# dremovd/PPO

Hardware: AMD Instinct MI355X
Metric: env-steps/sec (Pong-shaped synthetic, 256 envs/GPU) (higher is better)
Workload: dtype f32

## Files before the change

include/ppo_amd.h:

```cpp
#ifndef PPO_AMD_H
#define PPO_AMD_H

#include <stddef.h>
#include <stdint.h>

#ifdef __cplusplus
extern "C" {
#endif

#define PPO_OK 0
#define PPO_E_INVALID (-1)
#define PPO_E_HIP (-2)
#define PPO_E_ALIGN (-3)

#define PPO_TERM_NONE 0
#define PPO_TERM_U8 1
#define PPO_TERM_F32 2

#define PPO_SCAN_AUTO 0
#define PPO_SCAN_COLUMNS 1
#define PPO_SCAN_TILES 2

int ppo_version(void);
const char *ppo_last_error(void);
// ... 177 lines not shown
                      void *stream);
int ppo_accumulate_f32(float *dst, const float *src, int64_t n, void *stream);
int ppo_mask_mul_f32(float *w, const uint8_t *mask, int64_t n, void *stream);

size_t ppo_tvf_returns_workspace_bytes(int N, int A, int ND, int K, int C);
int ppo_tvf_returns_f32(const float *rewards, const uint8_t *dones, const float *value_samples, int N, int A, int V,
                        int K, int C, double gamma, const int32_t *n_eff, const int32_t *nd_index,
                        const int32_t *nd_of_n, int max_n, int ND, const int32_t *main_plan, const double *main_w,
                        const int32_t *tail_plan, const double *tail_w, const uint8_t *k_zero, void *workspace,
                        size_t workspace_bytes, float *out, void *stream);

int ppo_impala_stack_tail_supported(int channels, int h, int w);
int ppo_impala_stack_tail_forward_f32(const float *in, const float *const *packed_weights, const float *const *biases,
                                      float *a0, float *q0, float *a1, float *q1, int n_images, int channels, int h,
                                      int w, void *stream);
int ppo_impala_stack_tail_backward_f32(const float *g, const float *const *packed_weights_t, const float *const *masks,
                                       float *da1, float *g1, float *da0, float *g0, int n_images, int channels,
                                       int h, int w, void *stream);

int ppo_impala_stack_full_supported(int channels, int h, int w);
int ppo_impala_stack_chain_forward_f32(const float *in, const float *const *pre_packed_weights,
                                       const float *const *pre_biases, float *pre_a0, float *pre_q0, float *pre_a1,
                                       float *pre_q1, const float *const *packed_weights, const float *const *biases,
                                       float *pooled, uint8_t *argmax, float *a0, float *q0, float *a1, float *q1,
                                       int n_images, int channels, int h, int w, void *stream);
size_t ppo_impala_stack_chain_split_workspace_bytes(int n_images, int channels, int h, int w);
int ppo_impala_stack_chain_split_forward_f32(const float *in, const float *const *pre_packed_weights,
                                             const float *const *pre_biases, const float *const *packed_weights,
                                             const float *const *biases, float *q1, void *workspace, size_t workspace_bytes,
                                             int n_images, int channels, int h, int w, void *stream);
int ppo_impala_stack_full_backward_f32(const float *g, const float *const *packed_weights_t, const float *const *masks,
                                       const uint8_t *argmax, float *da1, float *g1, float *da0, float *g0, float *dc,
                                       float *g_prev, int n_images, int channels, int h, int w, void *stream);
int ppo_impala_stack_full_forward_f32(const float *in, const float *const *packed_weights, const float *const *biases,
                                      float *pooled, uint8_t *argmax, float *a0, float *q0, float *a1, float *q1,
                                      int n_images, int channels, int h, int w, void *stream);

int ppo_obs_moments_f64(const void *x, int is_u8, int B, int F, double *moments, void *stream);
int ppo_obs_rms_update_f64(const double *moments, double batch_count, double count, double *mean, double *var,
                           float *mu, float *std, int F, void *stream);
int ppo_obs_normalize_f32(const void *x, int is_u8, const float *mu, const float *std, float eps, float *out, int B,
                          int F, void *stream);

void *ppo_synth_env_create(int n_envs, int64_t obs_bytes, uint64_t seed, double p_done, int64_t env_offset,
                           int n_threads);
void ppo_synth_env_destroy(void *env);
int ppo_synth_env_reset(void *env, uint8_t *obs_out);
int ppo_synth_env_step(void *env, const int32_t *actions, uint8_t *obs_out, float *reward_out, uint8_t *done_out,
                       int32_t *time_out, float *ep_score_out, int32_t *ep_len_out);
int ppo_synth_env_step_upload(void *env, const int32_t *actions, uint8_t *obs_out, float *reward_out, uint8_t *done_out,
                              int32_t *time_out, float *ep_score_out, int32_t *ep_len_out, void *obs_dev, int n_chunks,
                              void *stream);
int ppo_synth_env_get_state(void *env, int64_t *steps_out, int32_t *time_out, float *score_out);
int ppo_synth_env_set_state(void *env, const int64_t *steps, const int32_t *time, const float *score, uint8_t *obs_out);

typedef struct ppo_mlp_net {
    const float *w1, *b1;
    const float *w2, *b2;
    const float *wh, *bh;
    int F, H, NH;
    int act;
} ppo_mlp_net;
typedef struct ppo_mlp_grads {
    float *dw1, *db1, *dw2, *db2, *dwh, *dbh;
    float *dlog_std;
    int n_log_std;
// ... 78 lines not shown
```

ppo_amd/_lib.py:

```python
import ctypes
import os
import threading

HERE = os.path.dirname(os.path.abspath(__file__))
LIB_PATH = os.environ.get("PPO_AMD_LIB") or os.path.join(HERE, "lib", "libppo_amd.so")

PPO_TERM_NONE, PPO_TERM_U8, PPO_TERM_F32 = 0, 1, 2
PPO_SCAN_AUTO, PPO_SCAN_COLUMNS, PPO_SCAN_TILES = 0, 1, 2
PPO_IN_NONE, PPO_IN_RELU, PPO_IN_U8 = 0, 1, 2

_vp = ctypes.c_void_p
_i = ctypes.c_int
_i64 = ctypes.c_int64
_d = ctypes.c_double
_f = ctypes.c_float
_sz = ctypes.c_size_t
_u64 = ctypes.c_uint64

SIGNATURES = {
    "ppo_version": (_i, []),
    "ppo_last_error": (ctypes.c_char_p, []),
    "ppo_gae_scan_f32": (_i, [_vp, _vp, _vp, _vp, _i, _vp, _vp, _i, _i, _i64, _d, _d, _d, _i, _vp]),
    "ppo_bootstrapped_returns_f32": (_i, [_vp, _vp, _i, _vp, _vp, _d, _vp, _i, _i, _i64, _vp]),
    "ppo_conv3x3_forward_f32": (_i, [_vp, _i, _vp, _vp, _vp, _vp, _i, _i, _i, _i, _i, _vp]),
# ... 28 lines not shown
    "ppo_synth_env_step_upload": (_i, [_vp, _vp, _vp, _vp, _vp, _vp, _vp, _vp, _vp, _i, _vp]),
    "ppo_synth_env_get_state": (_i, [_vp, _vp, _vp, _vp]),
    "ppo_synth_env_set_state": (_i, [_vp, _vp, _vp, _vp, _vp]),
    "ppo_ppo_loss_f32": (_i, [_vp, _i, _i, _i, _i, _vp, _vp, _vp, _vp, _vp, _f, _f, _f, _f, _vp, _vp, _vp, _vp]),
    "ppo_conv3x3_pool_forward_f32": (_i, [_vp, _i, _vp, _vp, _vp, _vp, _i, _i, _i, _i, _i, _vp]),
    "ppo_conv3x3_packed_floats": (_sz, [_i, _i, _i]),
    "ppo_conv3x3_pack_weights_f32": (_i, [_vp, _i, _vp]),
    "ppo_conv3x3_forward_packed_f32": (_i, [_vp, _i, _vp, _vp, _vp, _vp, _i, _i, _i, _i, _i, _vp]),
    "ppo_conv3x3_backward_data_packed_f32": (_i, [_vp, _vp, _vp, _vp, _vp, _i, _i, _i, _i, _i, _vp]),
    "ppo_conv3x3_pool_forward_packed_f32": (_i, [_vp, _i, _vp, _vp, _vp, _vp, _i, _i, _i, _i, _i, _vp]),
    "ppo_conv3x3_pool_forward_packed_indexed_f32": (_i, [_vp, _vp, _i, _vp, _vp, _vp, _vp, _i, _i, _i, _i, _i, _vp]),
    "ppo_conv1_pool_form": (_i, [_i]),
    "ppo_conv3x3_block_supported": (_i, [_i, _i, _i]),
    "ppo_conv3x3_block_forward_packed_f32": (_i, [_vp, _vp, _vp, _vp, _vp, _vp, _i, _i, _i, _i, _vp]),
    "ppo_conv3x3_backward_weight_slabs_f32": (_i, [_vp, _i, _vp, _vp, _sz, _i, _i, _i, _i, _i, _vp, _vp]),
    "ppo_conv3x3_backward_weight_pooled_supported": (_i, [_i, _i, _i, _i]),
    "ppo_conv3x3_backward_weight_slabs_pooled_f32": (_i, [_vp, _i, _vp, _vp, _vp, _sz, _i, _i, _i, _i, _i, _vp, _vp]),
    "ppo_conv3x3_backward_weight_slabs_pooled_indexed_f32": (_i, [_vp, _vp, _i, _vp, _vp, _vp, _sz, _i, _i, _i, _i, _i, _vp, _vp]),
    "ppo_conv3x3_backward_weight_slabs_batch_f32": (_i, [_vp, _i, _vp, _vp, _sz, _i, _i, _i, _i, _i, _i, _vp, _vp]),
    "ppo_conv3x3_backward_weight_slabs_batch_mixed_f32": (_i, [_vp, _vp, _vp, _vp, _sz, _i, _i, _i, _i, _i, _i, _vp, _vp]),
    "ppo_conv3x3_backward_weight_bf16x3_supported": (_i, [_i, _i, _i, _i]),
    "ppo_conv3x3_backward_weight_slabs_batch_bf16x3": (_i, [_vp, _vp, _vp, _vp, _sz, _i, _i, _i, _i, _i, _i, _vp, _vp]),
    "ppo_conv3x3_wgrad_reduce_f32": (_i, [_vp, _i, _vp]),
    "ppo_tanh_forward_f32": (_i, [_vp, _vp, _sz, _vp]),
    "ppo_tanh_backward_f32": (_i, [_vp, _vp, _vp, _sz, _vp]),
    "ppo_value_loss_f32": (_i, [_vp, _i, _i, _i, _i, _vp, _f, _i, _i, _i, _vp, _vp, _f, _f, _vp, _vp, _vp, _f, _u64, _u64, _vp]),
    "ppo_distil_loss_f32": (_i, [_vp, _i, _i, _i, _i, _i, _i, _i, _vp, _vp, _vp, _vp, _f, _f, _vp, _vp, _vp, _vp]),
    "ppo_gaussian_act_f32": (_i, [_vp, _i, _i, _i, _vp, _vp, _u64, _u64, _i, _vp, _vp, _vp, _vp, _i, _vp]),
    "ppo_gaussian_loss_f32": (_i, [_vp, _i, _i, _i, _i, _vp, _vp, _vp, _vp, _vp, _f, _f, _f, _vp, _vp, _vp, _vp, _vp]),
    "ppo_impala_stack_tail_supported": (_i, [_i, _i, _i]),
    "ppo_impala_stack_tail_forward_f32": (_i, [_vp, _vp, _vp, _vp, _vp, _vp, _vp, _i, _i, _i, _i, _vp]),
    "ppo_impala_stack_full_supported": (_i, [_i, _i, _i]),
    "ppo_impala_stack_full_backward_f32": (_i, [_vp] * 10 + [_i, _i, _i, _i, _vp]),
    "ppo_impala_stack_chain_forward_f32": (_i, [_vp] * 15 + [_i, _i, _i, _i, _vp]),
    "ppo_impala_stack_chain_split_workspace_bytes": (_sz, [_i, _i, _i, _i]),
    "ppo_impala_stack_chain_split_forward_f32": (_i, [_vp, _vp, _vp, _vp, _vp, _vp, _vp, _sz, _i, _i, _i, _i, _vp]),
    "ppo_impala_stack_full_forward_f32": (_i, [_vp, _vp, _vp, _vp, _vp, _vp, _vp, _vp, _vp, _i, _i, _i, _i, _vp]),
    "ppo_impala_stack_tail_backward_f32": (_i, [_vp, _vp, _vp, _vp, _vp, _vp, _vp, _i, _i, _i, _i, _vp]),
    "ppo_obs_moments_f64": (_i, [_vp, _i, _i, _i, _vp, _vp]),
    "ppo_obs_rms_update_f64": (_i, [_vp, _d, _d, _vp, _vp, _vp, _vp, _i, _vp]),
    "ppo_obs_normalize_f32": (_i, [_vp, _i, _vp, _vp, _f, _vp, _i, _i, _vp]),
    "ppo_adam_workspace_bytes": (_sz, []),
    "ppo_adam_step_f32": (_i, [_vp, _vp, _vp, _vp, _i64, _i64, _d, _d, _d, _d, _f, _f, _vp, _vp, _vp]),
    "ppo_adam_step_presummed_f32": (_i, [_vp, _vp, _vp, _vp, _i64, _i64, _d, _d, _d, _d, _f, _f, _vp, _i, _vp, _vp]),
    "ppo_impala_stack_tail_bf16x3_packed_bytes": (_sz, []),
    "ppo_impala_stack_tail_bf16x3_supported": (_i, [_i, _i, _i]),
    "ppo_impala_stack_tail_pack_bf16x3": (_i, [_vp, _vp, _i, _i, _vp]),
    "ppo_impala_stack_tail_pack_bf16x3_jobs": (_i, [_vp, _i, _vp]),
    "ppo_impala_stack_tail_forward_bf16x3": (_i, [_vp, _vp, _vp, _vp, _vp, _vp, _vp, _i, _i, _i, _i, _vp]),
    "ppo_impala_stack_tail_backward_bf16x3": (_i, [_vp, _vp, _vp, _vp, _vp, _vp, _vp, _i, _i, _i, _i, _vp]),
    "ppo_impala_stack_tail_bf16x3_sign_bytes": (_sz, [_i, _i, _i, _i]),
    "ppo_impala_stack_tail_forward_signs_bf16x3": (_i, [_vp, _vp, _vp, _vp, _vp, _vp, _vp, _vp, _i, _i, _i, _i, _vp]),
    "ppo_impala_stack_tail_backward_signs_bf16x3": (_i, [_vp, _vp, _vp, _vp, _vp, _vp, _vp, _i, _i, _i, _i, _vp]),
    "ppo_conv3x3_bf16x3_supported": (_i, [_i, _i, _i, _i]),
    "ppo_conv3x3_bf16x3_packed_bytes": (_sz, [_i, _i]),
    "ppo_conv3x3_pack_bf16x3_jobs": (_i, [_vp, _i, _vp]),
    "ppo_conv3x3_bf16x3": (_i, [_vp, _i, _vp, _vp, _vp, _i, _i, _i, _i, _i, _vp]),
    "ppo_conv3x3_pool_bf16x3_supported": (_i, [_i, _i, _i, _i]),
    "ppo_conv3x3_backward_weight_slabs_batch_bf16_split": (_i, [_vp, _vp, _vp, _vp, _sz, _i, _i, _i, _i, _i, _i, _i, _vp, _vp]),
    "ppo_conv3x3_bf16_split_packed_bytes": (_sz, [_i, _i, _i]),
    "ppo_conv3x3_pack_bf16_split": (_i, [_vp, _vp, _i, _i, _i, _i, _vp]),
    "ppo_conv3x3_bf16_split": (_i, [_vp, _i, _vp, _vp, _vp, _i, _i, _i, _i, _i, _i, _vp]),
    "ppo_conv3x3_pool_bf16x3": (_i, [_vp, _i, _vp, _vp, _vp, _vp, _i, _i, _i, _i, _i, _vp]),
    "ppo_mlp_supported": (_i, [_i, _i, _i]),
    "ppo_mlp_forward_f32": (_i, [_vp, _vp, _vp, _i, _vp, _vp, _vp, _vp]),
    "ppo_mlp_train_workspace_floats": (_sz, [_i, _i, _i, _i]),
# ... 109 lines not shown
```

ppo_amd/csrc/stack_fused.hip:

```cpp
#include <cstdlib>
#include <type_traits>

#include "common.h"
#include "conv_stage.h"
#include "mfma.h"

#ifndef PPO_TAIL_SPLIT
#define PPO_TAIL_SPLIT 2
#endif

namespace ppo {
namespace {

constexpr int kScrPitchS = 20;

struct StackTailArgs {
    const float *in;
    const float *w[4];
    const float *bias[4];
    const float *mask[4];
    float *save[4];
    int n_images;
};

// ... 445 lines not shown
        const int pc = p < H * W ? p : 0;
        lm.lofs[m] = G + pc - 1 + g * PLANE;
        lm.hi_l[m] = (pc % W == 0) ? 0.f : INFINITY;
        lm.hi_r[m] = (pc % W == W - 1) ? 0.f : INFINITY;
    }
}

template <int C, int H, int W, int MT, int NTOT, int NT, bool RELU_IN, bool GATED = false>
__device__ __forceinline__ void resident_conv(float *smem, int src_off, int dst_off, bool residual, const float *wpk,
                                              const float *bias, float *save, const LaneMap::T<MT> &lm, int n0, int lane,
                                              const float *mask = nullptr)
{
    constexpr int ROWS = H + 2, G = 4, PLANE_RAW = ROWS * W + 2 * G;
    constexpr int PLANE = PLANE_RAW + ((16 - PLANE_RAW % 32) + 32) % 32;
    constexpr int KS = 9 * (C / 4);
    const int g = lane >> 4;
    float wa[NT][KS];
    const float4 *pw = reinterpret_cast<const float4 *>(wpk);
#pragma unroll
    for (int s4 = 0; s4 < KS / 4; ++s4)
#pragma unroll
        for (int n = 0; n < NT; ++n) {
            const float4 v = pw[(s4 * NTOT + n0 + n) * 64 + lane];
            wa[n][4 * s4 + 0] = v.x;
            wa[n][4 * s4 + 1] = v.y;
            wa[n][4 * s4 + 2] = v.z;
            wa[n][4 * s4 + 3] = v.w;
        }
    float bias_r[NT][4];
#pragma unroll
    for (int n = 0; n < NT; ++n)
#pragma unroll
        for (int r = 0; r < 4; ++r) bias_r[n][r] = (GATED || !bias) ? 0.f : bias[(n0 + n) * 16 + g * 4 + r];
    float gate[GATED ? MT : 1][NT][4];
    if constexpr (GATED) {
        const __amdgpu_buffer_rsrc_t mask_b = buffer_of(mask);
#pragma unroll
        for (int m = 0; m < MT; ++m)
#pragma unroll
            for (int n = 0; n < NT; ++n)
#pragma unroll
                for (int r = 0; r < 4; ++r)
                    gate[m][n][r] = buffer_f32(mask_b, lm.pix[m] < H * W ? (((n0 + n) * 16 + g * 4 + r) * (H * W) + lm.pix[m]) * 4
                                                                         : kOutside);
    }

    __syncthreads();
    int base[MT];
#pragma unroll
    for (int m = 0; m < MT; ++m) base[m] = lm.lofs[m] + src_off;
    f32x4 acc[NT][MT];
#pragma unroll
    for (int n = 0; n < NT; ++n)
#pragma unroll
        for (int m = 0; m < MT; ++m) acc[n][m] = f32x4{0.f, 0.f, 0.f, 0.f};

    constexpr int SB = (MT * NT >= 4) ? 2 : 4;
    constexpr int NB = (KS + SB - 1) / SB;
    float raw[2][SB][MT];
    auto load_block = [&](int j, float (&r)[SB][MT]) {
#pragma unroll
        for (int u = 0; u < SB; ++u) {
            const int s = j * SB + u;
            if (s < KS) {
                const int tap = s / (C / 4), cs = s % (C / 4);
                const int tap_off = (tap / 3) * W + (tap % 3);
#pragma unroll
                for (int m = 0; m < MT; ++m) r[u][m] = smem[base[m] + cs * 4 * PLANE + tap_off];
            }
        }
    };
    load_block(0, raw[0]);
    static_for<0, NB>([&](auto jc) {
        constexpr int j = decltype(jc)::value;
        float bv[SB][MT];
#pragma unroll
        for (int u = 0; u < SB; ++u) {
            const int s = j * SB + u;
            if (s < KS) {
                const int kx = (s / (C / 4)) % 3;
#pragma unroll
                for (int m = 0; m < MT; ++m) {
                    float x = raw[j & 1][u][m];
                    if (kx != 1) {
                        const float hi = kx == 0 ? lm.hi_l[m] : lm.hi_r[m];
                        x = __builtin_amdgcn_fmed3f(x, RELU_IN ? 0.f : -hi, hi);
                    } else if (RELU_IN) {
                        x = relu1(x);
                    }
                    bv[u][m] = x;
                }
            }
        }
        __builtin_amdgcn_sched_barrier(0);
        if constexpr (j + 1 < NB) load_block(j + 1, raw[(j + 1) & 1]);
#pragma unroll
        for (int u = 0; u < SB; ++u) {
            const int s = j * SB + u;
            if (s < KS) {
#pragma unroll
                for (int m = 0; m < MT; ++m)
#pragma unroll
                    for (int n = 0; n < NT; ++n) acc[n][m] = mfma16(wa[n][s], bv[u][m], acc[n][m]);
            }
        }
        __builtin_amdgcn_sched_barrier(0);
    });
#pragma unroll
    for (int m = 0; m < MT; ++m) {
        if (lm.pix[m] < H * W) {
#pragma unroll
            for (int n = 0; n < NT; ++n)
#pragma unroll
                for (int r = 0; r < 4; ++r) {
                    const int co = (n0 + n) * 16 + g * 4 + r;
                    const int lo = dst_off + co * PLANE + G + W + lm.pix[m];
                    float val = acc[n][m][r] + bias_r[n][r];
                    if constexpr (GATED) val = gate[m][n][r] > 0.f ? val : 0.f;
                    if (residual) val = val + smem[lo];
                    smem[lo] = val;
                    if (save) save[(size_t)co * (H * W) + lm.pix[m]] = val;
                }
        }
    }
}

struct StackFullArgs {
    const float *in;
// ... 56 lines not shown
                const int u = u0 + sub;
                const int co = u / HO, yo = u % HO;
                if (sub < RPW && co < C) {
                    const float *src = smem + B_OFF + co * SI::PLANE + SI::G + WI + (2 * yo - 1) * WI + 2 * xo - 1;
                    float best;
                    int best_tap;
                    pool_window_lds<HI % 2 == 0, WI % 2 == 0>(src, WI, yo > 0, 2 * yo + 1 < HI, xo > 0, 2 * xo + 1 < WI, best, best_tap);
                    smem[X_OFF + co * SO::PLANE + SO::G + WO + yo * WO + xo] = best;
                    const size_t oi = out_img + ((size_t)co * HO + yo) * WO + xo;
                    if (a.pooled) a.pooled[oi] = best;
                    if (a.argmax) a.argmax[oi] = (uint8_t)best_tap;
                }
            }
        }
        const size_t out_img = (size_t)img * C * HO * WO;
#pragma unroll 1
        for (int layer = 0; layer < 4; ++layer) {
            const int odd = layer & 1;
            float *save = a.save[layer] ? a.save[layer] + out_img : nullptr;
            resident_conv<C, HO, WO, MTO, SO::NT, NT, true>(smem, odd ? Y_OFF : X_OFF, odd ? X_OFF : Y_OFF, odd != 0,
                                                            a.w[1 + layer], a.bias[1 + layer], save, lmo, n0, lane);
        }
    }
}

struct StackFullBwdArgs {
    const float *g;
    const float *w[5];
    const float *mask[4];
    const uint8_t *argmax;
    float *save[4];
    float *dc;
    float *g_prev;
    int n_images;
};

template <int C, int HI, int WI, int MTI, int HO, int WO, int MTO, int NW, int NSPLIT>
__global__ __launch_bounds__(NW * NSPLIT * 64) void stack_full_bwd_kernel(StackFullBwdArgs a)
{
    using SI = StackCfg<C, HI, WI, MTI, NW, NSPLIT>;
    using SO = StackCfg<C, HO, WO, MTO, NW, NSPLIT>;
    static_assert(2 * SO::LDS_MAP <= SI::LDS_MAP, "the small maps live inside the first big map's LDS");
    constexpr int NT = SI::NTL, WAVES = SI::WAVES, THREADS = WAVES * 64;
    constexpr int A_OFF = 0, B_OFF = SI::LDS_MAP, X_OFF = 0, Y_OFF = SO::LDS_MAP;
    extern __shared__ __align__(16) float smem[];
    const int tid = threadIdx.x, lane = tid & 63, l15 = lane & 15, g = lane >> 4;
    const int wave = tid >> 6, pixel_wave = wave % NW, n0 = (wave / NW) * NT;

    LaneMap::T<MTI> lmi;
    LaneMap::T<MTO> lmo;
    lane_map_init<HI, WI, SI::PLANE, SI::G, MTI>(lmi, pixel_wave, l15, g);
    lane_map_init<HO, WO, SO::PLANE, SO::G, MTO>(lmo, pixel_wave, l15, g);

    zero_lds<SI::LDS_MAP, THREADS>(smem + B_OFF, tid);

    for (int img = blockIdx.x; img < a.n_images; img += gridDim.x) {
        __syncthreads();
        zero_lds<2 * SO::LDS_MAP, THREADS>(smem + X_OFF, tid);
        __syncthreads();
        stage_band_chunk_dma<C, HO, WO, SO::ROWS, SO::PLANE, SO::G, WAVES>(a.g, img, 0, smem + X_OFF, tid);
        const size_t small_img = (size_t)img * C * HO * WO, big_img = (size_t)img * C * HI * WI;
#pragma unroll 1
        for (int layer = 0; layer < 4; ++layer) {
            const int odd = layer & 1;
            resident_conv<C, HO, WO, MTO, SO::NT, NT, false, true>(smem, odd ? Y_OFF : X_OFF, odd ? X_OFF : Y_OFF, odd != 0,
                                                                   a.w[layer], nullptr, a.save[layer] + small_img, lmo, n0,
                                                                   lane, a.mask[layer] + small_img);
        }
        __syncthreads();
        {
            const uint8_t *am = a.argmax + small_img;
            for (int e = tid; e < C * HI * WI; e += THREADS) {
                const int co = e / (HI * WI), r = e % (HI * WI);
                const int iy = r / WI, ix = r % WI;
                const int k = ix >> 1, oy0 = iy >> 1;
                const int ky0 = (iy & 1) ? 2 : 1;
                const bool has_oy1 = (iy & 1) && (oy0 + 1 < HO);
                const bool odd_x = ix & 1;
                const bool has_ox1 = odd_x && (k + 1 < WO);
                const int kx0 = odd_x ? 2 : 1;
                const float *gx = smem + X_OFF + co * SO::PLANE + SO::G + WO;
                const uint8_t *ac = am + co * (HO * WO);
                float sum = 0.f;
                {
                    const int i00 = oy0 * WO + k;
                    if (ac[i00] == ky0 * 3 + kx0) sum += gx[i00];
                    if (has_ox1 && ac[i00 + 1] == ky0 * 3 + 0) sum += gx[i00 + 1];
                }
                if (has_oy1) {
                    const int i10 = (oy0 + 1) * WO + k;
                    if (ac[i10] == kx0) sum += gx[i10];
                    if (has_ox1 && ac[i10 + 1] == 0) sum += gx[i10 + 1];
                }
                smem[B_OFF + co * SI::PLANE + SI::G + WI + r] = sum;
                a.dc[big_img + e] = sum;
            }
        }
        resident_conv<C, HI, WI, MTI, SI::NT, NT, false, false>(smem, B_OFF, A_OFF, false, a.w[4], nullptr,
                                                                a.g_prev + big_img, lmi, n0, lane);
    }
}

template <int C, int HI, int WI, int MTI, int HO, int WO, int MTO, int NW, int NSPLIT>
int launch_stack_full_bwd(const StackFullBwdArgs &args, hipStream_t st)
{
    using SI = StackCfg<C, HI, WI, MTI, NW, NSPLIT>;
    constexpr size_t kLds = 2 * (size_t)SI::LDS_MAP * 4;
    auto kern = stack_full_bwd_kernel<C, HI, WI, MTI, HO, WO, MTO, NW, NSPLIT>;
    static bool ready = false;
    if (!ready) {
        hipError_t e = hipFuncSetAttribute(reinterpret_cast<const void *>(kern), hipFuncAttributeMaxDynamicSharedMemorySize,
                                           (int)kLds);
        if (e != hipSuccess) return fail(PPO_E_HIP, "stack_full_bwd: hipFuncSetAttribute: %s", hipGetErrorString(e));
        ready = true;
    }
    const int grid = args.n_images < 256 ? args.n_images : 256;
    hipLaunchKernelGGL(kern, dim3(grid), dim3(SI::WAVES * 64), kLds, st, args);
    return check_launch("stack_full_bwd_kernel");
}

template <int C, int HI, int WI, int MTI, int HO, int WO, int MTO, int NW, int NSPLIT>
int launch_stack_full(const StackFullArgs &args, hipStream_t st)
{
    using SI = StackCfg<C, HI, WI, MTI, NW, NSPLIT>;
    constexpr size_t kLds = 2 * (size_t)SI::LDS_MAP * 4;
    auto kern = stack_full_kernel<C, HI, WI, MTI, HO, WO, MTO, NW, NSPLIT>;
    static bool ready = false;
    if (!ready) {
        hipError_t e = hipFuncSetAttribute(reinterpret_cast<const void *>(kern), hipFuncAttributeMaxDynamicSharedMemorySize,
                                           (int)kLds);
        if (e != hipSuccess) return fail(PPO_E_HIP, "stack_full: hipFuncSetAttribute: %s", hipGetErrorString(e));
        ready = true;
// ... 310 lines not shown
            args.pre_w[l] = pre_packed_weights[l];
            args.pre_bias[l] = pre_biases[l];
        }
    }
    args.pre_save[0] = pre_a0;
    args.pre_save[1] = pre_q0;
    args.pre_save[2] = pre_a1;
    args.pre_save[3] = pre_q1;
    args.has_pre = 1;
    args.pooled = pooled;
    args.argmax = argmax;
    args.save[0] = a0;
    args.save[1] = q0;
    args.save[2] = a1;
    args.save[3] = q1;
    args.n_images = n_images;
    if (channels == 32 && h == 21 && w == 21)
        return launch_stack_full<32, 21, 21, 7, 11, 11, 2, 4, 2>(args, as_stream(stream));
    if (channels == 32 && h == 16 && w == 16)
        return launch_stack_full<32, 16, 16, 4, 8, 8, 1, 4, 2>(args, as_stream(stream));
    return fail(PPO_E_INVALID, "ppo_impala_stack_chain_forward_f32: no kernel for %d channels at %dx%d", channels, h, w);
}

extern "C" int ppo_impala_stack_full_backward_f32(const float *g, const float *const *packed_weights_t,
                                                  const float *const *masks, const uint8_t *argmax, float *da1, float *g1,
                                                  float *da0, float *g0, float *dc, float *g_prev, int n_images,
                                                  int channels, int h, int w, void *stream)
{
    using namespace ppo;
    if (n_images < 0) return fail(PPO_E_INVALID, "ppo_impala_stack_full_backward_f32: negative batch");
    if (n_images == 0) return PPO_OK;
    if (!g || !packed_weights_t || !masks || !argmax || !da1 || !g1 || !da0 || !g0 || !dc || !g_prev)
        return fail(PPO_E_INVALID, "ppo_impala_stack_full_backward_f32: null pointer");
    StackFullBwdArgs args;
    args.g = g;
    for (int l = 0; l < 5; ++l) {
        if (!packed_weights_t[l] || (l < 4 && !masks[l]))
            return fail(PPO_E_INVALID, "ppo_impala_stack_full_backward_f32: null weights / mask of layer %d", l);
        if (!aligned(packed_weights_t[l], 16))
            return fail(PPO_E_ALIGN, "ppo_impala_stack_full_backward_f32: packed weights must be 16-byte aligned");
        args.w[l] = packed_weights_t[l];
        if (l < 4) args.mask[l] = masks[l];
    }
    args.argmax = argmax;
    args.save[0] = da1;
    args.save[1] = g1;
    args.save[2] = da0;
    args.save[3] = g0;
    args.dc = dc;
    args.g_prev = g_prev;
    args.n_images = n_images;
    if (channels == 32 && h == 21 && w == 21)
        return launch_stack_full_bwd<32, 21, 21, 7, 11, 11, 2, 4, 2>(args, as_stream(stream));
    if (channels == 32 && h == 16 && w == 16)
        return launch_stack_full_bwd<32, 16, 16, 4, 8, 8, 1, 4, 2>(args, as_stream(stream));
    return fail(PPO_E_INVALID, "ppo_impala_stack_full_backward_f32: no kernel for %d channels at %dx%d", channels, h, w);
}

extern "C" size_t ppo_impala_stack_chain_split_workspace_bytes(int n_images, int channels, int h, int w)
{
    const size_t slots = (size_t)n_images * 2 * channels * h * w * sizeof(float);
    const size_t flags = ((size_t)n_images * 2 * sizeof(uint32_t) + 15) & ~(size_t)15;
    return slots + flags + 16;
}

extern "C" int ppo_impala_stack_chain_split_forward_f32(const float *in, const float *const *pre_packed_weights,
                                                        const float *const *pre_biases,
                                                        const float *const *packed_weights, const float *const *biases,
                                                        float *q1, void *workspace, size_t workspace_bytes, int n_images,
                                                        int channels, int h, int w, void *stream)
{
    using namespace ppo;
    if (n_images < 0) return fail(PPO_E_INVALID, "ppo_impala_stack_chain_split_forward_f32: negative batch");
    if (n_images == 0) return PPO_OK;
    if (!in || !pre_packed_weights || !pre_biases || !packed_weights || !biases || !q1 || !workspace)
        return fail(PPO_E_INVALID, "ppo_impala_stack_chain_split_forward_f32: null pointer");
    if (!(channels == 32 && h == 21 && w == 21))
        return fail(PPO_E_INVALID, "ppo_impala_stack_chain_split_forward_f32: no kernel for %d channels at %dx%d", channels, h, w);
    if (workspace_bytes < ppo_impala_stack_chain_split_workspace_bytes(n_images, channels, h, w) || !aligned(workspace, 16))
        return fail(PPO_E_INVALID, "ppo_impala_stack_chain_split_forward_f32: workspace too small or misaligned");
    ChainSplitArgs args;
    args.in = in;
    for (int l = 0; l < 5; ++l) {
        if (!packed_weights[l] || !biases[l] || (l < 4 && (!pre_packed_weights[l] || !pre_biases[l])))
            return fail(PPO_E_INVALID, "ppo_impala_stack_chain_split_forward_f32: null weights / bias of layer %d", l);
        if (!aligned(packed_weights[l], 16) || (l < 4 && !aligned(pre_packed_weights[l], 16)))
            return fail(PPO_E_ALIGN, "ppo_impala_stack_chain_split_forward_f32: packed weights must be 16-byte aligned");
        args.w[l] = packed_weights[l];
        args.bias[l] = biases[l];
// ... 21 lines not shown
```

ppo_amd/models.py:

```python
import ctypes
import math
import os
from collections import OrderedDict
from typing import Dict, Optional

import numpy as np
import torch

from . import _lib

IN_NONE, IN_RELU, IN_U8 = _lib.PPO_IN_NONE, _lib.PPO_IN_RELU, _lib.PPO_IN_U8
_ALIGN = 4
FUSE_POOL_STACKS = int(os.environ.get("PPO_AMD_FUSE_POOL", "7"))
WGRAD_BATCH_LAUNCH = int(os.environ.get("PPO_AMD_WGRAD_BATCH_LAUNCH", "1"))
WGRAD_POOLED_DY = int(os.environ.get("PPO_AMD_WGRAD_POOLED_DY", "1"))
WGRAD_RIDE = int(os.environ.get("PPO_AMD_WGRAD_RIDE", "1"))
SPLIT_WGRAD = int(os.environ.get("PPO_AMD_SPLIT_WGRAD", "1"))
SPLIT_CONV = int(os.environ.get("PPO_AMD_SPLIT_CONV", "1"))
PACKED_WEIGHTS = int(os.environ.get("PPO_AMD_PACKED_WEIGHTS", "1"))
ADAM_SCATTER = int(os.environ.get("PPO_AMD_ADAM_SCATTER", "0"))
FUSE_STACK_TAIL = int(os.environ.get("PPO_AMD_FUSE_STACK_TAIL", "1"))
FUSE_STACK_FULL = int(os.environ.get("PPO_AMD_FUSE_STACK_FULL", "1"))
FUSE_STACK_CHAIN = int(os.environ.get("PPO_AMD_FUSE_STACK_CHAIN", "1"))
CHAIN_SPLIT = int(os.environ.get("PPO_AMD_CHAIN_SPLIT", "1"))
CHAIN_SPLIT_MAX_BATCH = 128
FUSE_STACK_FULL_BWD = int(os.environ.get("PPO_AMD_FUSE_STACK_FULL_BWD", "0"))
FUSE_STACK_TAIL_BWD = int(os.environ.get("PPO_AMD_FUSE_STACK_TAIL_BWD", "7"))
FUSE_STACK16_MIN_BATCH = int(os.environ.get("PPO_AMD_FUSE_STACK16_MIN_BATCH", "192"))
FUSE_BLOCK = int(os.environ.get("PPO_AMD_FUSE_BLOCK", "1"))
FUSE_MLP = int(os.environ.get("PPO_AMD_FUSE_MLP", "1"))
GATHER_IN_CONV = int(os.environ.get("PPO_AMD_GATHER_IN_CONV", "1"))
HEAD_NAMES = ("policy_head", "value_head", "advantage_head", "tvf_head")


def _p(t):
    return None if t is None else t.data_ptr()


def _normed_conv(cin, cout, scale=1.0):
    m = torch.nn.Conv2d(cin, cout, 3, padding=1)
    with torch.no_grad():
        m.weight.data *= scale / m.weight.norm(dim=(1, 2, 3), p=2, keepdim=True)
        m.bias.data *= 0
    return m.weight.data, m.bias.data


def _normed_linear(fin, fout, scale=1.0):
    m = torch.nn.Linear(fin, fout)
    with torch.no_grad():
        m.weight.data *= scale / m.weight.norm(dim=1, p=2, keepdim=True)
        m.bias.data *= 0
    return m.weight.data, m.bias.data


def _custom_linear(fin, fout, scale=1.0, bias=True):
    m = torch.nn.Linear(fin, fout, bias=bias)
    with torch.no_grad():
        if m.bias is not None:
            m.bias.data *= 0
        torch.nn.init.orthogonal_(m.weight.data, gain=scale)
# ... 1029 lines not shown
                x, dy, wname, n, c, hh, ww = carry.pop()
                wgrad(x, IN_NONE, dy, wname, n, c, c, hh, ww)

        def wgrad_blocks(problems, n, c, hh, ww):
            if not WGRAD_BATCH_LAUNCH or len(problems) > 4:
                flush_carry()
                for x, dy, wname in problems:
                    wgrad(x, IN_RELU, dy, wname, n, c, c, hh, ww)
                return
            relu = [1] * len(problems)
            if carry and carry[-1][3:] == (n, c, hh, ww):
                x, dy, wname = carry.pop()[:3]
                problems = list(problems) + [(x, dy, wname)]
                relu.append(0)
            flush_carry()
            nbytes = lib.ppo_conv3x3_wgrad_workspace_bytes(c, c)
            wss = [self._ws("wgrad_ws_" + wname, nbytes) for _x, _dy, wname in problems]
            k = len(problems)
            n_slabs = ctypes.c_int(0)
            ins = (ctypes.c_void_p * k)(*[x.data_ptr() for x, _d, _w in problems])
            dys = (ctypes.c_void_p * k)(*[dy.data_ptr() for _x, dy, _w in problems])
            wsp = (ctypes.c_void_p * k)(*[ws.data_ptr() for ws in wss])
            if split_wgrad(IN_RELU, c, c, hh, ww):
                args_ = ("ppo_conv3x3_backward_weight_slabs_batch_bf16x3", ins, (ctypes.c_int * k)(*relu), dys, wsp, nbytes, k, n,
                         c, c, hh, ww, ctypes.addressof(n_slabs))
            elif k > 4:
                args_ = ("ppo_conv3x3_backward_weight_slabs_batch_mixed_f32", ins, (ctypes.c_int * k)(*relu), dys, wsp, nbytes, k, n,
                         c, c, hh, ww, ctypes.addressof(n_slabs))
            else:
                args_ = ("ppo_conv3x3_backward_weight_slabs_batch_f32", ins, IN_RELU, dys, wsp, nbytes, k, n, c, c, hh, ww,
                         ctypes.addressof(n_slabs))
            slab_launch(args_, n_slabs, [(wname, ws) for (_x, _dy, wname), ws in zip(problems, wss)], c, c)

        for si in reversed(range(len(sp.stacks))):
            cin, cout, hh, ww, ho, wo = sp.stacks[si]
            full_w = self._stack_full_bwd_ptrs(si, cin, cout, hh, ww) if si > 0 else None
            tail_w = self._stack_tail_bwd_ptrs(si, cout, ho, wo) if full_w is None else None
            split = full_w is None and self.split_bf16 and (si, 1) in self._pk16
            fused = full_w is not None or tail_w is not None or split
            if fused:
                b0, b1 = f"encoder.stacks.{si}.blocks.0", f"encoder.stacks.{si}.blocks.1"
                p_in, a0, q0, a1 = acts[f"q{si}_0_in"], acts[f"a{si}_0"], acts[f"q{si}_1_in"], acts[f"a{si}_1"]
                da1, g1, da0, g0 = (self._buf(nm, (B, cout, ho, wo)) for nm in
                                    (f"g{si}_1_da", f"g{si}_1_in", f"g{si}_0_da", f"g{si}_0_in"))
                masks = (ctypes.c_void_p * 4)(a1.data_ptr(), q0.data_ptr(), a0.data_ptr(), p_in.data_ptr())
                if full_w is not None:
                    dc = self._buf(f"g{si}_dc", (B, cout, hh, ww))
                    g_prev = self._buf(f"g{si - 1}_top", (B, cin, hh, ww))
                    self._call("ppo_impala_stack_full_backward_f32", _p(g), full_w, masks, _p(acts[f"idx{si}"]), _p(da1), _p(g1),
                               _p(da0), _p(g0), _p(dc), _p(g_prev), B, cout, hh, ww)
                elif split and acts.get(f"signs{si}") is not None:
                    self._call("ppo_impala_stack_tail_backward_signs_bf16x3", _p(g), _p(self._pk16[(si, 1)]), acts[f"signs{si}"],
                               _p(da1), _p(g1), _p(da0), _p(g0), B, cout, ho, wo)
                elif split:
                    self._call("ppo_impala_stack_tail_backward_bf16x3", _p(g), _p(self._pk16[(si, 1)]), masks, _p(da1), _p(g1),
                               _p(da0), _p(g0), B, cout, ho, wo)
                else:
                    self._call("ppo_impala_stack_tail_backward_f32", _p(g), tail_w, masks, _p(da1), _p(g1), _p(da0), _p(g0),
                               B, cout, ho, wo)
                wgrad_blocks([(a1, g, b1 + ".conv1"), (q0, da1, b1 + ".conv0"), (a0, g1, b0 + ".conv1"),
                              (p_in, da0, b0 + ".conv0")], B, cout, ho, wo)
                if full_w is not None:
                    wgrad(acts[f"in{si}"], IN_NONE, dc, f"encoder.stacks.{si}.firstconv", B, cin, cout, hh, ww)
                    g = g_prev
                    continue
                g = g0
            defer = WGRAD_BATCH_LAUNCH and sp.n_block * 2 <= 4
            problems = []
            for bi in (() if fused else reversed(range(sp.n_block))):
                base = f"encoder.stacks.{si}.blocks.{bi}"
                q_in, a = acts[f"q{si}_{bi}_in"], acts[f"a{si}_{bi}"]
                if defer:
                    problems.append((a, g, base + ".conv1"))
# ... 23 lines not shown
                    and mode == IN_NONE and sp.n_block == 2 and sp.stacks[si - 1][1] == cin \
                    and tuple(sp.stacks[si - 1][4:6]) == (hh, ww):
                carry.append((x_in, dc, f"encoder.stacks.{si}.firstconv", B, cin, hh, ww))
            else:
                wgrad(x_in, mode, dc, f"encoder.stacks.{si}.firstconv", B, cin, cout, hh, ww)
            if si > 0:
                g = self._buf(f"g{si - 1}_top", (B, cin, hh, ww))
                fc = f"encoder.stacks.{si}.firstconv"
                if self.split_bf16 and (fc, 1) in self._pk16:
                    self._call("ppo_conv3x3_bf16x3", _p(dc), 0, _p(self._pk16[(fc, 1)]), None, _p(g), B, cout, cin, hh, ww)
                else:
                    self._call(self._bwd_data_fn(fc), _p(dc), _p(self._bwd_w(fc)),
                               None, None, _p(g), B, cin, cout, hh, ww)
        flush_carry()
        if jobs:
            table = (_lib.WgradJob * len(jobs))(*jobs)
            self._call("ppo_conv3x3_wgrad_reduce_f32", ctypes.addressof(table), len(jobs))

    def _stack_full_bwd_ptrs(self, si, cin, cout, h, w):
        if not (FUSE_STACK_FULL_BWD and FUSE_STACK_TAIL) or self.spec.n_block != 2 or cin != cout \
                or not self.lib.ppo_impala_stack_full_supported(cout, h, w):
            return None
        cached = self._tail_ptrs.get(("full_bwd", si))
        if cached is None:
            names = [f"encoder.stacks.{si}.blocks.{bi}.conv{ci}" for bi in (1, 0) for ci in (1, 0)]
            names.append(f"encoder.stacks.{si}.firstconv")
            pks = [self._pk.get((n, 1)) for n in names]
            if any(pk is None for pk in pks):
                return None
            cached = (ctypes.c_void_p * 5)(*[pk.data_ptr() for pk in pks])
            self._tail_ptrs[("full_bwd", si)] = cached
        return cached

    def _stack_tail_bwd_ptrs(self, si, cout, ho, wo):
        if not (FUSE_STACK_TAIL and FUSE_STACK_TAIL_BWD >> si & 1) or self.spec.n_block != 2 \
                or not self.lib.ppo_impala_stack_tail_supported(cout, ho, wo):
            return None
        cached = self._tail_ptrs.get(("bwd", si))
        if cached is None:
            names = [f"encoder.stacks.{si}.blocks.{bi}.conv{ci}" for bi in (1, 0) for ci in (1, 0)]
            pks = [self._pk.get((n, 1)) for n in names]
            if any(pk is None for pk in pks):
                return None
            cached = (ctypes.c_void_p * 4)(*[pk.data_ptr() for pk in pks])
            self._tail_ptrs[("bwd", si)] = cached
        return cached

    def _bwd_data_fn(self, wname):
        return "ppo_conv3x3_backward_data_packed_f32" if (wname, 1) in self._pk else "ppo_conv3x3_backward_data_f32"

    def _bwd_w(self, wname):
        return self._pk.get((wname, 1), self.params[wname + ".weight"])

    def takes_obs_index(self, obs) -> bool:
        if self.encoder_kind != "impala" or obs.dtype != torch.uint8 or self.obs_norm is not None or not GATHER_IN_CONV:
            return False
        cin, cout, h, w, _ho, _wo = self.spec.stacks[0]
        return bool(FUSE_POOL_STACKS & 1) and self._pk.get(("encoder.stacks.0.firstconv", 0)) is not None \
            and bool(WGRAD_POOLED_DY) \
            and bool(self.lib.ppo_conv3x3_backward_weight_pooled_supported(cin, cout, h, w))

    @staticmethod
    def _minibatch_rows(prev_state, index, obs_indexed) -> int:
        if obs_indexed:
            if index is None:
                raise ValueError("obs_indexed=True needs the index that prev_state is read through")
# ... 342 lines not shown
```

Measured before the change: 97350.

## Fuse adjacent IMPALA stacks' backward into one chained resident kernel

Adds a chained backward entry point that, after a stack's full backward (residual blocks, maxpool unpool, firstconv data-grad), keeps the resulting gradient resident in LDS and runs the previous stack's four residual-block backward convolutions in the same kernel. This avoids a separate launch and a round trip of the intermediate gradient through global memory. It also preloads argmax bytes into registers and then into LDS to avoid scattered global byte reads, and defers the gate mask load into the middle of the k-loop to overlap its latency. It is used by default when batch is at least 192 and split_bf16 is off. The cost is longer per-block kernels and a new alignment requirement on argmax.

```diff
diff --git a/include/ppo_amd.h b/include/ppo_amd.h
--- a/include/ppo_amd.h
+++ b/include/ppo_amd.h
@@ -233,6 +233,11 @@
 int ppo_impala_stack_full_backward_f32(const float *g, const float *const *packed_weights_t, const float *const *masks,
                                        const uint8_t *argmax, float *da1, float *g1, float *da0, float *g0, float *dc,
                                        float *g_prev, int n_images, int channels, int h, int w, void *stream);
+int ppo_impala_stack_chain_backward_f32(const float *g, const float *const *packed_weights_t, const float *const *masks,
+                                        const uint8_t *argmax, float *da1, float *g1, float *da0, float *g0, float *dc,
+                                        float *g_prev, const float *const *post_packed_weights_t,
+                                        const float *const *post_masks, float *post_da1, float *post_g1, float *post_da0,
+                                        float *post_g0, int n_images, int channels, int h, int w, void *stream);
 int ppo_impala_stack_full_forward_f32(const float *in, const float *const *packed_weights, const float *const *biases,
                                       float *pooled, uint8_t *argmax, float *a0, float *q0, float *a1, float *q1,
                                       int n_images, int channels, int h, int w, void *stream);
diff --git a/ppo_amd/_lib.py b/ppo_amd/_lib.py
--- a/ppo_amd/_lib.py
+++ b/ppo_amd/_lib.py
@@ -84,6 +84,7 @@
     "ppo_impala_stack_tail_forward_f32": (_i, [_vp, _vp, _vp, _vp, _vp, _vp, _vp, _i, _i, _i, _i, _vp]),
     "ppo_impala_stack_full_supported": (_i, [_i, _i, _i]),
     "ppo_impala_stack_full_backward_f32": (_i, [_vp] * 10 + [_i, _i, _i, _i, _vp]),
+    "ppo_impala_stack_chain_backward_f32": (_i, [_vp] * 16 + [_i, _i, _i, _i, _vp]),
     "ppo_impala_stack_chain_forward_f32": (_i, [_vp] * 15 + [_i, _i, _i, _i, _vp]),
     "ppo_impala_stack_chain_split_workspace_bytes": (_sz, [_i, _i, _i, _i]),
     "ppo_impala_stack_chain_split_forward_f32": (_i, [_vp, _vp, _vp, _vp, _vp, _vp, _vp, _sz, _i, _i, _i, _i, _vp]),
diff --git a/ppo_amd/csrc/stack_fused.hip b/ppo_amd/csrc/stack_fused.hip
--- a/ppo_amd/csrc/stack_fused.hip
+++ b/ppo_amd/csrc/stack_fused.hip
@@ -501,8 +501,11 @@
     for (int n = 0; n < NT; ++n)
 #pragma unroll
         for (int r = 0; r < 4; ++r) bias_r[n][r] = (GATED || !bias) ? 0.f : bias[(n0 + n) * 16 + g * 4 + r];
+    constexpr int SB = (MT * NT >= 4) ? 2 : 4;
+    constexpr int NB = (KS + SB - 1) / SB;
+    constexpr int GATE_AT = (GATED && MT * NT * 4 > 16) ? NB / 2 : -1;
     float gate[GATED ? MT : 1][NT][4];
-    if constexpr (GATED) {
+    auto load_gate = [&]() {
         const __amdgpu_buffer_rsrc_t mask_b = buffer_of(mask);
 #pragma unroll
         for (int m = 0; m < MT; ++m)
@@ -512,7 +515,8 @@
                 for (int r = 0; r < 4; ++r)
                     gate[m][n][r] = buffer_f32(mask_b, lm.pix[m] < H * W ? (((n0 + n) * 16 + g * 4 + r) * (H * W) + lm.pix[m]) * 4
                                                                          : kOutside);
-    }
+    };
+    if constexpr (GATED && GATE_AT < 0) load_gate();
 
     __syncthreads();
     int base[MT];
@@ -524,8 +528,6 @@
 #pragma unroll
         for (int m = 0; m < MT; ++m) acc[n][m] = f32x4{0.f, 0.f, 0.f, 0.f};
 
-    constexpr int SB = (MT * NT >= 4) ? 2 : 4;
-    constexpr int NB = (KS + SB - 1) / SB;
     float raw[2][SB][MT];
     auto load_block = [&](int j, float (&r)[SB][MT]) {
 #pragma unroll
@@ -563,6 +565,7 @@
         }
         __builtin_amdgcn_sched_barrier(0);
         if constexpr (j + 1 < NB) load_block(j + 1, raw[(j + 1) & 1]);
+        if constexpr (j == GATE_AT) load_gate();
 #pragma unroll
         for (int u = 0; u < SB; ++u) {
             const int s = j * SB + u;
@@ -685,6 +688,10 @@
     float *save[4];
     float *dc;
     float *g_prev;
+    const float *post_w[4];
+    const float *post_mask[4];
+    float *post_save[4];
+    int has_post;
     int n_images;
 };
 
@@ -694,6 +701,7 @@
     using SI = StackCfg<C, HI, WI, MTI, NW, NSPLIT>;
     using SO = StackCfg<C, HO, WO, MTO, NW, NSPLIT>;
     static_assert(2 * SO::LDS_MAP <= SI::LDS_MAP, "the small maps live inside the first big map's LDS");
+    static_assert(C * HO * WO <= SO::LDS_MAP * 4, "the argmax bytes of an image fit the second small map");
     constexpr int NT = SI::NTL, WAVES = SI::WAVES, THREADS = WAVES * 64;
     constexpr int A_OFF = 0, B_OFF = SI::LDS_MAP, X_OFF = 0, Y_OFF = SO::LDS_MAP;
     extern __shared__ __align__(16) float smem[];
@@ -713,6 +721,14 @@
         __syncthreads();
         stage_band_chunk_dma<C, HO, WO, SO::ROWS, SO::PLANE, SO::G, WAVES>(a.g, img, 0, smem + X_OFF, tid);
         const size_t small_img = (size_t)img * C * HO * WO, big_img = (size_t)img * C * HI * WI;
+        constexpr int AM_WORDS = C * HO * WO / 4, AM_PER = (AM_WORDS + THREADS - 1) / THREADS;
+        static_assert(C * HO * WO % 4 == 0, "an image's argmax bytes are whole words (the entry points check the base)");
+        uint32_t am_r[AM_PER];
+#pragma unroll
+        for (int k = 0; k < AM_PER; ++k) {
+            const int i = tid + k * THREADS;
+            am_r[k] = reinterpret_cast<const uint32_t *>(a.argmax + small_img)[i < AM_WORDS ? i : 0];
+        }
 #pragma unroll 1
         for (int layer = 0; layer < 4; ++layer) {
             const int odd = layer & 1;
@@ -721,8 +737,14 @@
                                                                    lane, a.mask[layer] + small_img);
         }
         __syncthreads();
+        const uint8_t *am = reinterpret_cast<const uint8_t *>(smem + Y_OFF);
+#pragma unroll
+        for (int k = 0; k < AM_PER; ++k) {
+            const int i = tid + k * THREADS;
+            if (i < AM_WORDS) reinterpret_cast<uint32_t *>(smem + Y_OFF)[i] = am_r[k];
+        }
+        __syncthreads();
         {
-            const uint8_t *am = a.argmax + small_img;
             for (int e = tid; e < C * HI * WI; e += THREADS) {
                 const int co = e / (HI * WI), r = e % (HI * WI);
                 const int iy = r / WI, ix = r % WI;
@@ -749,8 +771,21 @@
                 a.dc[big_img + e] = sum;
             }
         }
+        if (a.has_post) {
+            __syncthreads();
+            zero_lds<SI::LDS_MAP, THREADS>(smem + A_OFF, tid);
+        }
         resident_conv<C, HI, WI, MTI, SI::NT, NT, false, false>(smem, B_OFF, A_OFF, false, a.w[4], nullptr,
                                                                 a.g_prev + big_img, lmi, n0, lane);
+        if (a.has_post) {
+#pragma unroll 1
+            for (int layer = 0; layer < 4; ++layer) {
+                const int odd = layer & 1;
+                resident_conv<C, HI, WI, MTI, SI::NT, NT, false, true>(smem, odd ? B_OFF : A_OFF, odd ? A_OFF : B_OFF, odd != 0,
+                                                                       a.post_w[layer], nullptr, a.post_save[layer] + big_img,
+                                                                       lmi, n0, lane, a.post_mask[layer] + big_img);
+            }
+        }
     }
 }
 
@@ -1127,6 +1162,7 @@
     if (n_images == 0) return PPO_OK;
     if (!g || !packed_weights_t || !masks || !argmax || !da1 || !g1 || !da0 || !g0 || !dc || !g_prev)
         return fail(PPO_E_INVALID, "ppo_impala_stack_full_backward_f32: null pointer");
+    if (!aligned(argmax, 4)) return fail(PPO_E_ALIGN, "ppo_impala_stack_full_backward_f32: argmax must be 4-byte aligned");
     StackFullBwdArgs args;
     args.g = g;
     for (int l = 0; l < 5; ++l) {
@@ -1144,12 +1180,66 @@
     args.save[3] = g0;
     args.dc = dc;
     args.g_prev = g_prev;
+    for (int l = 0; l < 4; ++l) {
+        args.post_w[l] = nullptr;
+        args.post_mask[l] = nullptr;
+        args.post_save[l] = nullptr;
+    }
+    args.has_post = 0;
     args.n_images = n_images;
     if (channels == 32 && h == 21 && w == 21)
         return launch_stack_full_bwd<32, 21, 21, 7, 11, 11, 2, 4, 2>(args, as_stream(stream));
     if (channels == 32 && h == 16 && w == 16)
         return launch_stack_full_bwd<32, 16, 16, 4, 8, 8, 1, 4, 2>(args, as_stream(stream));
     return fail(PPO_E_INVALID, "ppo_impala_stack_full_backward_f32: no kernel for %d channels at %dx%d", channels, h, w);
+}
+
+extern "C" int ppo_impala_stack_chain_backward_f32(const float *g, const float *const *packed_weights_t,
+                                                   const float *const *masks, const uint8_t *argmax, float *da1, float *g1,
+                                                   float *da0, float *g0, float *dc, float *g_prev,
+                                                   const float *const *post_packed_weights_t, const float *const *post_masks,
+                                                   float *post_da1, float *post_g1, float *post_da0, float *post_g0,
+                                                   int n_images, int channels, int h, int w, void *stream)
+{
+    using namespace ppo;
+    if (n_images < 0) return fail(PPO_E_INVALID, "ppo_impala_stack_chain_backward_f32: negative batch");
+    if (n_images == 0) return PPO_OK;
+    if (!g || !packed_weights_t || !masks || !argmax || !da1 || !g1 || !da0 || !g0 || !dc || !g_prev || !post_packed_weights_t
+        || !post_masks || !post_da1 || !post_g1 || !post_da0 || !post_g0)
+        return fail(PPO_E_INVALID, "ppo_impala_stack_chain_backward_f32: null pointer");
+    if (!aligned(argmax, 4)) return fail(PPO_E_ALIGN, "ppo_impala_stack_chain_backward_f32: argmax must be 4-byte aligned");
+    StackFullBwdArgs args;
+    args.g = g;
+    for (int l = 0; l < 5; ++l) {
+        if (!packed_weights_t[l] || (l < 4 && (!masks[l] || !post_packed_weights_t[l] || !post_masks[l])))
+            return fail(PPO_E_INVALID, "ppo_impala_stack_chain_backward_f32: null weights / mask of layer %d", l);
+        if (!aligned(packed_weights_t[l], 16) || (l < 4 && !aligned(post_packed_weights_t[l], 16)))
+            return fail(PPO_E_ALIGN, "ppo_impala_stack_chain_backward_f32: packed weights must be 16-byte aligned");
+        args.w[l] = packed_weights_t[l];
+        if (l < 4) {
+            args.mask[l] = masks[l];
+            args.post_w[l] = post_packed_weights_t[l];
+            args.post_mask[l] = post_masks[l];
+        }
+    }
+    args.argmax = argmax;
+    args.save[0] = da1;
+    args.save[1] = g1;
+    args.save[2] = da0;
+    args.save[3] = g0;
+    args.dc = dc;
+    args.g_prev = g_prev;
+    args.post_save[0] = post_da1;
+    args.post_save[1] = post_g1;
+    args.post_save[2] = post_da0;
+    args.post_save[3] = post_g0;
+    args.has_post = 1;
+    args.n_images = n_images;
+    if (channels == 32 && h == 21 && w == 21)
+        return launch_stack_full_bwd<32, 21, 21, 7, 11, 11, 2, 4, 2>(args, as_stream(stream));
+    if (channels == 32 && h == 16 && w == 16)
+        return launch_stack_full_bwd<32, 16, 16, 4, 8, 8, 1, 4, 2>(args, as_stream(stream));
+    return fail(PPO_E_INVALID, "ppo_impala_stack_chain_backward_f32: no kernel for %d channels at %dx%d", channels, h, w);
 }
 
 extern "C" size_t ppo_impala_stack_chain_split_workspace_bytes(int n_images, int channels, int h, int w)
diff --git a/ppo_amd/models.py b/ppo_amd/models.py
--- a/ppo_amd/models.py
+++ b/ppo_amd/models.py
@@ -26,6 +26,7 @@
 CHAIN_SPLIT_MAX_BATCH = 128
 FUSE_STACK_FULL_BWD = int(os.environ.get("PPO_AMD_FUSE_STACK_FULL_BWD", "0"))
 FUSE_STACK_TAIL_BWD = int(os.environ.get("PPO_AMD_FUSE_STACK_TAIL_BWD", "7"))
+FUSE_CHAIN_BWD_MIN_BATCH = 192
 FUSE_STACK16_MIN_BATCH = int(os.environ.get("PPO_AMD_FUSE_STACK16_MIN_BATCH", "192"))
 FUSE_BLOCK = int(os.environ.get("PPO_AMD_FUSE_BLOCK", "1"))
 FUSE_MLP = int(os.environ.get("PPO_AMD_FUSE_MLP", "1"))
@@ -1121,13 +1122,47 @@
                          ctypes.addressof(n_slabs))
             slab_launch(args_, n_slabs, [(wname, ws) for (_x, _dy, wname), ws in zip(problems, wss)], c, c)
 
+        chained = None
         for si in reversed(range(len(sp.stacks))):
             cin, cout, hh, ww, ho, wo = sp.stacks[si]
+            chain_w = self._stack_chain_bwd_ptrs(si, B) if chained is None else None
+            if chain_w is not None:
+                pi = si - 1
+                names = ("_1_da", "_1_in", "_0_da", "_0_in")
+                da1, g1, da0, g0 = (self._buf(f"g{si}{nm}", (B, cout, ho, wo)) for nm in names)
+                pda1, pg1, pda0, pg0 = (self._buf(f"g{pi}{nm}", (B, cin, hh, ww)) for nm in names)
+                dc = self._buf(f"g{si}_dc", (B, cout, hh, ww))
+                g_prev = self._buf(f"g{pi}_top", (B, cin, hh, ww))
+                p_in, a0, q0, a1 = acts[f"q{si}_0_in"], acts[f"a{si}_0"], acts[f"q{si}_1_in"], acts[f"a{si}_1"]
+                masks = (ctypes.c_void_p * 4)(a1.data_ptr(), q0.data_ptr(), a0.data_ptr(), p_in.data_ptr())
+                pmasks = (ctypes.c_void_p * 4)(*[acts[k].data_ptr() for k in
+                                                 (f"a{pi}_1", f"q{pi}_1_in", f"a{pi}_0", f"q{pi}_0_in")])
+                self._call("ppo_impala_stack_chain_backward_f32", _p(g), chain_w[0], masks, _p(acts[f"idx{si}"]), _p(da1),
+                           _p(g1), _p(da0), _p(g0), _p(dc), _p(g_prev), chain_w[1], pmasks, _p(pda1), _p(pg1), _p(pda0),
+                           _p(pg0), B, cout, hh, ww)
+                b0, b1 = f"encoder.stacks.{si}.blocks.0", f"encoder.stacks.{si}.blocks.1"
+                wgrad_blocks([(a1, g, b1 + ".conv1"), (q0, da1, b1 + ".conv0"), (a0, g1, b0 + ".conv1"),
+                              (p_in, da0, b0 + ".conv0")], B, cout, ho, wo)
+                if WGRAD_RIDE and WGRAD_BATCH_LAUNCH:
+                    carry.append((acts[f"in{si}"], dc, f"encoder.stacks.{si}.firstconv", B, cin, hh, ww))
+                else:
+                    wgrad(acts[f"in{si}"], IN_NONE, dc, f"encoder.stacks.{si}.firstconv", B, cin, cout, hh, ww)
+                g = g_prev
+                chained = (pi, pg0)
+                continue
             full_w = self._stack_full_bwd_ptrs(si, cin, cout, hh, ww) if si > 0 else None
             tail_w = self._stack_tail_bwd_ptrs(si, cout, ho, wo) if full_w is None else None
             split = full_w is None and self.split_bf16 and (si, 1) in self._pk16
             fused = full_w is not None or tail_w is not None or split
-            if fused:
+            if chained is not None and chained[0] == si:
+                fused, full_w = True, None
+                b0, b1 = f"encoder.stacks.{si}.blocks.0", f"encoder.stacks.{si}.blocks.1"
+                p_in, a0, q0, a1 = acts[f"q{si}_0_in"], acts[f"a{si}_0"], acts[f"q{si}_1_in"], acts[f"a{si}_1"]
+                wgrad_blocks([(a1, g, b1 + ".conv1"), (q0, self._buf(f"g{si}_1_da", (B, cout, ho, wo)), b1 + ".conv0"),
+                              (a0, self._buf(f"g{si}_1_in", (B, cout, ho, wo)), b0 + ".conv1"),
+                              (p_in, self._buf(f"g{si}_0_da", (B, cout, ho, wo)), b0 + ".conv0")], B, cout, ho, wo)
+                g = chained[1]
+            elif fused:
                 b0, b1 = f"encoder.stacks.{si}.blocks.0", f"encoder.stacks.{si}.blocks.1"
                 p_in, a0, q0, a1 = acts[f"q{si}_0_in"], acts[f"a{si}_0"], acts[f"q{si}_1_in"], acts[f"a{si}_1"]
                 da1, g1, da0, g0 = (self._buf(nm, (B, cout, ho, wo)) for nm in
@@ -1217,6 +1252,26 @@
             self._tail_ptrs[("full_bwd", si)] = cached
         return cached
 
+    def _stack_chain_bwd_ptrs(self, si, batch):
+        if si < 1 or self.split_bf16 or batch < FUSE_CHAIN_BWD_MIN_BATCH or self.spec.n_block != 2 \
+                or not (FUSE_STACK_TAIL and FUSE_STACK_TAIL_BWD >> si & 1 and FUSE_STACK_TAIL_BWD >> (si - 1) & 1):
+            return None
+        cin, cout, h, w, _ho, _wo = self.spec.stacks[si]
+        if cin != cout or self.spec.stacks[si - 1][1] != cin or tuple(self.spec.stacks[si - 1][4:6]) != (h, w) \
+                or not self.lib.ppo_impala_stack_full_supported(cout, h, w):
+            return None
+        cached = self._tail_ptrs.get(("chain_bwd", si))
+        if cached is None:
+            names = [f"encoder.stacks.{s_}.blocks.{bi}.conv{ci}" for s_ in (si, si - 1) for bi in (1, 0) for ci in (1, 0)]
+            names.insert(4, f"encoder.stacks.{si}.firstconv")
+            pks = [self._pk.get((n, 1)) for n in names]
+            if any(pk is None for pk in pks):
+                return None
+            cached = ((ctypes.c_void_p * 5)(*[pk.data_ptr() for pk in pks[:5]]),
+                      (ctypes.c_void_p * 4)(*[pk.data_ptr() for pk in pks[5:]]))
+            self._tail_ptrs[("chain_bwd", si)] = cached
+        return cached
+
     def _stack_tail_bwd_ptrs(self, si, cout, ho, wo):
         if not (FUSE_STACK_TAIL and FUSE_STACK_TAIL_BWD >> si & 1) or self.spec.n_block != 2 \
                 or not self.lib.ppo_impala_stack_tail_supported(cout, ho, wo):
```

After: 98540 (median of 6 runs). 1.01x the previous value.
